# zipnn/zipnn

Hardware: NVIDIA H100
Metric: compress+decompress GB/s on bf16 tensors (higher is better)
Workload: dtype u8

## Files before the change

__graft_entry__.py:

```python
import os
import sys

ROOT = os.path.dirname(os.path.abspath(__file__))
if ROOT not in sys.path:
    sys.path.insert(0, ROOT)


def build() -> None:
    from zipnn_b200 import _native
    _native.build()
    from oracle import oracle as O
    O.build(ref=True)
    import subprocess
    emu = os.path.join(ROOT, "tests", "host_emu")
    subprocess.check_call(["g++", "-O2", "-shared", "-fPIC", "-o", os.path.join(emu, "libemu_serial.so"),
                           os.path.join(emu, "emu_serial.cpp")])
    import zipnn_b200
    _native.lib()


def smoke() -> None:
    import numpy as np
    import torch
    from oracle import oracle as O
    from zipnn_b200 import ZipNN, _native

    assert torch.cuda.is_available(), "smoke() needs a GPU"
    before = _native.launch_count()
    rng = np.random.default_rng(1234)
    for dt, n in ((torch.bfloat16, 300001), (torch.float32, 70001), (torch.float16, 4099), (torch.float8_e4m3fn, 200000)):
        x = torch.from_numpy(rng.standard_normal(n, dtype=np.float32) * np.float32(0.02 if dt != torch.float8_e4m3fn else 0.5)).to(dt)
        z = ZipNN(input_format="torch")
        stream = z.compress(x.cuda())
        plan = ZipNN(input_format="torch").plan(x)
        raw = x.contiguous().view(torch.uint8).numpy()
        want = O.zipnn_compress(plan["header"], raw, plan["num_buf"], plan["bit_reorder"], plan["byte_reorder"],
                                plan["chunk"], plan["threshold"], threads=2)
        got = stream.cpu().numpy()
        assert got.size == want.size and np.array_equal(got, want), f"stream mismatch for {dt}"
        back = ZipNN(input_format="torch").decompress(stream)
        assert back.is_cuda and back.dtype == dt
        assert np.array_equal(back.cpu().contiguous().view(torch.uint8).numpy(), raw), f"round trip mismatch for {dt}"
    torch.cuda.synchronize()
    launched = _native.launch_count() - before
    assert launched > 0
    print(f"smoke ok: 4 dtypes byte-exact vs oracle, {launched} kernel launches from libzipnn_b200.so")


if __name__ == "__main__":
# ... 4 lines not shown
```

zipnn_b200/csrc/api_compress.inc:

```

namespace {
constexpr size_t kHdrMax = 4096;
struct EncWs {
  size_t hdr_off, types_off, sizes_off, itemoff_off, saves_off, part_off, part_bytes, hist_off, total;
};
inline EncWs enc_ws_layout(size_t n, int G, size_t chunk) {
  EncWs L;
  const uint64_t nitems = (uint64_t)G * num_chunks(n, chunk);
  L.hdr_off = kCtrlBytes;
  L.types_off = L.hdr_off + kHdrMax;
  L.sizes_off = round_up(L.types_off + nitems, 256);
  L.itemoff_off = round_up(L.sizes_off + 4 * nitems, 256);
  L.saves_off = round_up(L.itemoff_off + 8 * nitems, 256);
  L.part_off = round_up(L.saves_off + sizeof(EncSave) * nitems, 256);
  L.part_bytes = 8 * (size_t)G * ((num_chunks(n, chunk) + kScanItems - 1) / kScanItems);
  L.hist_off = round_up(L.part_off + L.part_bytes, 256);
  L.total = L.hist_off + 2048 * nitems + 256;
  return L;
}

template <int G>
int launch_encode(const uint8_t* in, size_t n, uint32_t chunk, uint64_t K, int bits_mode, double thr, uint8_t* ws,
                  const EncWs& L, uint32_t hdr_len, uint8_t* out, cudaStream_t st) {
  Ctrl* ctrl = (Ctrl*)ws;
  uint8_t* types = ws + L.types_off;
  uint32_t* sizes = (uint32_t*)(ws + L.sizes_off);
  uint64_t* item_off = (uint64_t*)(ws + L.itemoff_off);
  EncSave* saves = (EncSave*)(ws + L.saves_off);
  const int sms = sm_count_cached();
  uint16_t* hist = (uint16_t*)(ws + L.hist_off);
  {
    const size_t smem = sizeof(HistSmem<G>);
    int per_sm = 1;
    if (smem > 48 * 1024) ZB_CUDA(cudaFuncSetAttribute(k_encode_hist<G>, cudaFuncAttributeMaxDynamicSharedMemorySize, (int)smem));
    ZB_CUDA(cudaOccupancyMaxActiveBlocksPerMultiprocessor(&per_sm, k_encode_hist<G>, kEncThreads, smem));
    if (per_sm < 1) per_sm = 1;
    const int blocks = (int)std::min<uint64_t>(K, (uint64_t)sms * per_sm);
    ScopedTimer tm(kKEncodeStats, st);
    k_encode_hist<G><<<blocks, kEncThreads, smem, st>>>(in, n, chunk, K, bits_mode, hist);
    ZB_LAUNCHED();
  }
  {
    const size_t smem = sizeof(TableWarp) * kTableWarps;
    const uint64_t nitems = (uint64_t)G * K;
    const int blocks = (int)std::min<uint64_t>((nitems + kTableWarps - 1) / kTableWarps, (uint64_t)sms * 16);
    ScopedTimer tm(kKEncodeTable, st);
    ZB_CUDA(cudaMemsetAsync(ws + L.part_off, 0, L.part_bytes, st));
    k_encode_table<G><<<blocks, kTableWarps * 32, smem, st>>>(hist, n, chunk, K, thr, types, sizes, saves,
                                                              (unsigned long long*)(ws + L.part_off));
    ZB_LAUNCHED();
  }
  {
    ScopedTimer tm(kKEncodeScan, st);
    const unsigned nblk = (unsigned)((K + kScanItems - 1) / kScanItems);
    k_encode_scan<<<(unsigned)G * nblk, kScanThreads, 0, st>>>(sizes, types, G, K, ws + L.hdr_off, hdr_len, out, item_off, ctrl,
                                                            (const unsigned long long*)(ws + L.part_off));
    ZB_LAUNCHED();
  }
  if (chunk % (64u * G) != 0) {
    int per_sm = 1;
    ZB_CUDA(cudaOccupancyMaxActiveBlocksPerMultiprocessor(&per_sm, k_encode_write<G>, kEncThreads, 0));
    if (per_sm < 1) per_sm = 1;
    const int blocks = (int)std::min<uint64_t>((uint64_t)G * K, (uint64_t)sms * per_sm);
    ScopedTimer tm(kKEncodeWriteRagged, st);
    k_encode_write<G><<<blocks, kEncThreads, 0, st>>>(in, n, chunk, K, bits_mode, types, sizes, saves, item_off, out, 0);
    ZB_LAUNCHED();
    return ZIPNN_B200_OK;
  }
  {
    int per_sm = 1;
    ZB_CUDA(cudaOccupancyMaxActiveBlocksPerMultiprocessor(&per_sm, k_encode_write_warp<G>, kWbWarps * 32, 0));
    if (per_sm < 1) per_sm = 1;
    const int blocks = (int)std::min<uint64_t>(K, (uint64_t)sms * per_sm);
    ScopedTimer tm(kKEncodeWrite, st);
    k_encode_write_warp<G><<<blocks, kWbWarps * 32, 0, st>>>(in, n, chunk, K, bits_mode, types, sizes, saves, item_off, out);
    ZB_LAUNCHED();
  }
  if ((n % chunk) % (64u * G) != 0) {
// ... 134 lines not shown
    L.part_at[i] = at;
    at += items[i].n ? enc_ws_layout(items[i].n, items[i].num_buf, items[i].chunk).part_bytes : 0;
  }
  L.zero_bytes = at - L.ctrl_off;
  at = round_up(at, 256);
  for (int i = 0; i < n; i++) {
    L.slice_at[i] = at;
    if (items[i].n) {
      const EncWs W = enc_ws_layout(items[i].n, items[i].num_buf, items[i].chunk);
      at += round_up(is_single(i) ? W.total : W.total - W.types_off, 256);
    }
  }
  L.total = at;
  return ZIPNN_B200_OK;
}

template <int G>
int launch_encode_batch(const EncTensor* d_t, uint32_t m, const uint64_t* d_start, const uint64_t* h_start, cudaStream_t st) {
  auto batch = [&](int q) { EncBatch b; b.t = d_t; b.start = d_start + (size_t)q * (m + 1); b.n = m; return b; };
  auto total = [&](int q) { return h_start[(size_t)q * (m + 1) + m]; };
  const int sms = sm_count_cached();
  {
    const size_t smem = sizeof(HistSmem<G>);
    int per_sm = 1;
    if (smem > 48 * 1024) ZB_CUDA(cudaFuncSetAttribute(k_encode_hist_batch<G>, cudaFuncAttributeMaxDynamicSharedMemorySize, (int)smem));
    ZB_CUDA(cudaOccupancyMaxActiveBlocksPerMultiprocessor(&per_sm, k_encode_hist_batch<G>, kEncThreads, smem));
    if (per_sm < 1) per_sm = 1;
    const int blocks = (int)std::max<uint64_t>(1, std::min<uint64_t>(total(0), (uint64_t)sms * per_sm));
    ScopedTimer tm(kKEncodeStats, st);
    k_encode_hist_batch<G><<<blocks, kEncThreads, smem, st>>>(batch(0));
    ZB_LAUNCHED();
  }
  {
    const size_t smem = sizeof(TableWarp) * kTableWarps;
    const int blocks = (int)std::max<uint64_t>(1, std::min<uint64_t>((total(1) + kTableWarps - 1) / kTableWarps, (uint64_t)sms * 16));
    ScopedTimer tm(kKEncodeTable, st);
    k_encode_table_batch<G><<<blocks, kTableWarps * 32, smem, st>>>(batch(1));
    ZB_LAUNCHED();
  }
  {
    ScopedTimer tm(kKEncodeScan, st);
    k_encode_scan_batch<<<(unsigned)total(2), kScanThreads, 0, st>>>(batch(2));
    ZB_LAUNCHED();
  }
  {
    int per_sm = 1;
    ZB_CUDA(cudaOccupancyMaxActiveBlocksPerMultiprocessor(&per_sm, k_encode_write_warp<G, EncBatch>, kWbWarps * 32, 0));
    if (per_sm < 1) per_sm = 1;
    const int blocks = (int)std::max<uint64_t>(1, std::min<uint64_t>(total(3), (uint64_t)sms * per_sm));
    ScopedTimer tm(kKEncodeWrite, st);
    k_encode_write_warp<G, EncBatch><<<blocks, kWbWarps * 32, 0, st>>>(nullptr, 0, 0, 0, 0, nullptr, nullptr, nullptr, nullptr, nullptr, batch(3));
    ZB_LAUNCHED();
  }
  if (total(4)) {
    int per_sm = 1;
    ZB_CUDA(cudaOccupancyMaxActiveBlocksPerMultiprocessor(&per_sm, k_encode_write<G, EncBatch>, kEncThreads, 0));
    if (per_sm < 1) per_sm = 1;
    const int blocks = (int)std::min<uint64_t>(total(4), (uint64_t)sms * per_sm);
    ScopedTimer tm(kKEncodeWriteRagged, st);
    k_encode_write<G, EncBatch><<<blocks, kEncThreads, 0, st>>>(nullptr, 0, 0, 0, 0, nullptr, nullptr, nullptr, nullptr, nullptr, 0, batch(4));
    ZB_LAUNCHED();
  }
  return ZIPNN_B200_OK;
}
}

extern "C" int zipnn_b200_compress_batch_workspace_size(const zipnn_b200_compress_item* items, int n, size_t* out) {
  if (!out) return ZIPNN_B200_E_ARG;
// ... 86 lines not shown
```

zipnn_b200/csrc/encode.cuh:

```cuda
#pragma once
#include "common.cuh"
#include "stage1.cuh"

#include <type_traits>

namespace zb {

struct EncSave {
  uint8_t nb[256];
  uint8_t hdr[128];
  uint32_t hsize;
  uint32_t sbytes[4];
  uint32_t lg;
  uint32_t pad[2];
};
static_assert(sizeof(EncSave) == 416, "EncSave layout");

constexpr int kEncThreads = 256;

struct EncTensor {
  const uint8_t* in;
  uint8_t* out;
  const uint8_t* hdr;
  uint64_t n, K;
  uint32_t chunk, hdr_len;
  int G, bits_mode;
  double thr;
  Ctrl* ctrl;
  unsigned long long* partials;
  uint8_t* types;
  uint32_t* sizes;
  uint64_t* item_off;
  EncSave* saves;
  uint16_t* hist;
};
// ... 100 lines not shown
      }
      if ((q & 1) == 0) continue;
      __syncthreads();
      for (int g = 0; g < G; g++) {
        uint32_t sum = 0;
#pragma unroll
        for (int r = 0; r < R; r++) {
          const int rr = (r + tid) % R;
          sum += S.rep[g][tid][rr];
          S.rep[g][tid][rr] = 0;
        }
        uint16_t* h = hist + (((uint64_t)g * K + c) * 4 + (q - 1)) * 256 + tid;
        h[0] = (uint16_t)(sum & 0xFFFFu);
        h[256] = (uint16_t)(sum >> 16);
      }
      __syncthreads();
    }
  }
}

template <int G>
__global__ void __launch_bounds__(kEncThreads) k_encode_hist(const uint8_t* __restrict__ in, uint64_t n, uint32_t chunk,
                                                             uint64_t K, int bits_mode, uint16_t* __restrict__ hist) {
  encode_hist<G>(in, n, chunk, K, bits_mode, hist, NoBatch{});
}

template <int G>
__global__ void __launch_bounds__(kEncThreads, G == 1 ? 2 : 3) k_encode_hist_batch(EncBatch B) {
  encode_hist<G>(nullptr, 0, 0, 0, 0, nullptr, B);
}

constexpr uint64_t kScanItems = 2048;

struct __align__(16) TableWarp {
  uint32_t total[256];
  uint8_t nb[256];
  uint8_t nzsym[256];
  TreeScratch tree;
};
constexpr int kTableWarps = 4;

__device__ void warp_block_decision(TableWarp& S, const uint16_t* __restrict__ hist, uint32_t plen, uint32_t cap, double thr,
                                    uint8_t* type_out, uint32_t* size_out, EncSave* save) {
  const int lane = threadIdx.x & 31;
  uint32_t* total = S.total;
  uint32_t largest = 0;
  int max_sym = -1;
  for (int s = lane; s < 256; s += 32) {
    const uint32_t t = (uint32_t)__ldg(hist + s) + __ldg(hist + 256 + s) + __ldg(hist + 512 + s) + __ldg(hist + 768 + s);
    total[s] = t;
    largest = max(largest, t);
    if (t) max_sym = s;
  }
#pragma unroll
  for (int o = 16; o; o >>= 1) {
    largest = max(largest, __shfl_xor_sync(0xffffffffu, largest, o));
    max_sym = max(max_sym, __shfl_xor_sync(0xffffffffu, max_sym, o));
  }
  __syncwarp();
  uint32_t stored = 0;
  bool huf = false;
  if (plen == 0 || plen > (uint32_t)kHufBlockMax) {
  } else if (largest == plen) {
    stored = huf_block_decision(true, nullptr, 0, plen, cap, thr);
    if (stored && lane == 0) {
      save->hdr[0] = (uint8_t)max_sym;
      save->hsize = 0;
    }
  } else if (largest <= (plen >> 7) + 4) {
  } else {
    huf = true;
  }
  if (huf) {
    TreeScratch& T = S.tree;
    uint8_t* nz = S.nzsym;
    int k = 0;
    for (int base = 0; base < 256; base += 32) {
      const int s = base + lane;
      const bool p = total[s] != 0;
      const uint32_t m = __ballot_sync(0xffffffffu, p);
      if (p) nz[k + __popc(m & ((1u << lane) - 1u))] = (uint8_t)s;
      k += __popc(m);
    }
    __syncwarp();
    for (int i = lane; i < k; i += 32) {
      const uint32_t c = total[nz[i]];
      int rank = 0;
      for (int j = 0; j < k; j++) {
        const uint32_t cj = total[nz[j]];
        rank += (cj > c) || (cj == c && j < i);
      }
      T.cnt[rank] = c;
      T.sym[rank] = nz[i];
    }
    __syncwarp();
    int lg = 0, hsize = -1;
    if (lane == 0) {
      const int want = fse_pick_log(kHufLogDefault, plen, (uint32_t)max_sym, 1);
      lg = huf_lengths_from_sorted(T, k - 1, want, S.nb);
      hsize = huf_write_table(T, S.nb, max_sym, lg);
    }
    lg = __shfl_sync(0xffffffffu, lg, 0);
    hsize = __shfl_sync(0xffffffffu, hsize, 0);
    __syncwarp();
    if (hsize > 0 && (uint32_t)hsize + 12 < plen) {
      uint32_t bits[4] = {0, 0, 0, 0};
      for (int s = lane; s <= max_sym; s += 32) {
        const uint32_t l = S.nb[s];
#pragma unroll
        for (int q = 0; q < 4; q++) bits[q] += (uint32_t)__ldg(hist + 256 * q + s) * l;
      }
#pragma unroll
      for (int q = 0; q < 4; q++)
#pragma unroll
        for (int o = 16; o; o >>= 1) bits[q] += __shfl_xor_sync(0xffffffffu, bits[q], o);
      stored = huf_block_decision(false, bits, hsize, plen, cap, thr);
      if (stored) {
        for (int s = lane; s < 256; s += 32) save->nb[s] = S.nb[s];
        for (int i = lane; i < hsize; i += 32) save->hdr[i] = T.hdr[i];
        if (lane == 0) {
          save->hsize = (uint32_t)hsize;
          save->lg = (uint32_t)lg;
#pragma unroll
          for (int q = 0; q < 4; q++) save->sbytes[q] = (bits[q] >> 3) + 1;
        }
      }
    }
  }
  if (lane == 0) {
    *type_out = stored ? 1 : 0;
    *size_out = stored ? stored : plen;
  }
}

template <int G>
__device__ __forceinline__ void encode_table_item(TableWarp& S, const uint16_t* __restrict__ hist, uint64_t n, uint32_t chunk, uint64_t K,
                                                  double thr, uint8_t* types, uint32_t* sizes, EncSave* saves,
                                                  unsigned long long* partials, const int lane, uint64_t item) {
  {
    const int g = (int)(item / K);
    const uint64_t c = item - (uint64_t)g * K;
    const uint32_t chunk_len = (c == K - 1) ? (uint32_t)(n - c * (uint64_t)chunk) : chunk;
    warp_block_decision(S, hist + item * 1024, plane_len(chunk_len, G, g), chunk, thr, types + item, sizes + item, saves + item);
    __syncwarp();
    if (lane == 0) atomicAdd(partials + (uint64_t)g * ((K + kScanItems - 1) / kScanItems) + c / kScanItems, (unsigned long long)sizes[item]);
  }
}

template <int G>
__global__ void __launch_bounds__(kTableWarps * 32) k_encode_table(const uint16_t* __restrict__ hist, uint64_t n, uint32_t chunk,
                                                                   uint64_t K, double thr, uint8_t* types, uint32_t* sizes,
                                                                   EncSave* saves, unsigned long long* partials) {
  extern __shared__ __align__(1024) unsigned char smem_raw[];
  TableWarp& S = reinterpret_cast<TableWarp*>(smem_raw)[threadIdx.x >> 5];
  const int lane = threadIdx.x & 31;
  const uint64_t nitems = (uint64_t)G * K;
  for (uint64_t item = (uint64_t)blockIdx.x * kTableWarps + (threadIdx.x >> 5); item < nitems;
       item += (uint64_t)gridDim.x * kTableWarps)
    encode_table_item<G>(S, hist, n, chunk, K, thr, types, sizes, saves, partials, lane, item);
}

constexpr int kScanThreads = 256;

__device__ __forceinline__ void encode_scan_block(const uint32_t* __restrict__ sizes, const uint8_t* __restrict__ types, int G, uint64_t K,
                                                  const uint8_t* __restrict__ hdr_dev, uint32_t hdr_len, uint8_t* out, uint64_t* item_off,
                                                  Ctrl* ctrl, const unsigned long long* __restrict__ partials, uint32_t bid) {
  __shared__ uint64_t warp_tot[kScanThreads / 32];
  __shared__ uint64_t red[kScanThreads / 32][3];
  const int tid = threadIdx.x, lane = tid & 31, warp = tid >> 5;
  const uint64_t nitems = (uint64_t)G * K;
  const uint64_t nblk = (K + kScanItems - 1) / kScanItems;
  const int g = (int)(bid / nblk);
  const uint64_t blk = bid - (uint64_t)g * nblk;
  uint64_t s_groups = 0, s_blocks = 0, s_all = 0;
  for (uint64_t i = tid; i < (uint64_t)G * nblk; i += kScanThreads) {
    const uint64_t v = partials[i];
    const uint64_t gi = i / nblk;
    s_all += v;
    if (gi < (uint64_t)g) s_groups += v;
    if (gi == (uint64_t)g && i - gi * nblk < blk) s_blocks += v;
  }
#pragma unroll
  for (int o = 16; o; o >>= 1) {
    s_groups += __shfl_xor_sync(0xffffffffu, s_groups, o);
    s_blocks += __shfl_xor_sync(0xffffffffu, s_blocks, o);
    s_all += __shfl_xor_sync(0xffffffffu, s_all, o);
  }
  if (lane == 0) { red[warp][0] = s_groups; red[warp][1] = s_blocks; red[warp][2] = s_all; }
  __syncthreads();
  s_groups = s_blocks = s_all = 0;
  for (int w = 0; w < kScanThreads / 32; w++) { s_groups += red[w][0]; s_blocks += red[w][1]; s_all += red[w][2]; }
// ... 588 lines not shown
            asm volatile("red.shared.or.b32 [%0+4], %1;" ::"r"(sa), "r"(w1) : "memory");
            asm volatile("{ .reg .pred p; setp.ne.u32 p, %1, 0; @p red.shared.or.b32 [%0+8], %1; }" ::"r"(sa), "r"(w2) : "memory");
            off += l[r];
          }
          __syncwarp();
          st[g].B += tile_bits;
          wb_flush(bitbuf, st[g], lane);
        }
      }
        };
    do_tile(std::false_type{}, ntiles - 1);
    for (uint32_t ti = ntiles - 1; ti-- > 0;) do_tile(std::true_type{}, ti);
#pragma unroll
    for (int g = 0; g < G; g++) {
      if (S.item[g].type == 1 && S.item[g].size > 1) {
        uint32_t* bitbuf = S.bitbuf[warp][g];
        if (lane == 0) bitbuf[(st[g].B - 32 * st[g].flushed) >> 5] |= 1u << (st[g].B & 31);
        __syncwarp();
        const uint32_t first_byte = max(4 * st[g].flushed, st[g].a);
        const uint32_t end_byte = st[g].a + S.item[g].sbytes[s];
        for (uint32_t bb = first_byte + lane; bb < end_byte; bb += 32) {
          const uint32_t rel = bb - 4 * st[g].flushed;
          st[g].gaddr[bb - st[g].a] = (uint8_t)(bitbuf[rel >> 2] >> (8 * (rel & 3)));
        }
        __syncwarp();
      }
    }
  }
}

template <int G>
__global__ void __launch_bounds__(kTableWarps * 32) k_encode_table_batch(EncBatch B) {
  extern __shared__ __align__(1024) unsigned char smem_raw[];
  TableWarp& S = reinterpret_cast<TableWarp*>(smem_raw)[threadIdx.x >> 5];
  const int lane = threadIdx.x & 31;
  const uint64_t total = B.start[B.n];
  for (uint64_t w = (uint64_t)blockIdx.x * kTableWarps + (threadIdx.x >> 5); w < total; w += (uint64_t)gridDim.x * kTableWarps) {
    const uint32_t i = batch_find(B.start, B.n, w);
    const EncTensor& T = B.t[i];
    encode_table_item<G>(S, T.hist, T.n, T.chunk, T.K, T.thr, T.types, T.sizes, T.saves, T.partials, lane, w - B.start[i]);
  }
}

__global__ void __launch_bounds__(kScanThreads) k_encode_scan_batch(EncBatch B) {
  const uint32_t i = batch_find(B.start, B.n, blockIdx.x);
  const EncTensor& T = B.t[i];
  if (T.K == 0) {
    for (uint32_t j = threadIdx.x; j < T.hdr_len; j += kScanThreads)
      T.out[j] = (j >= 24 && j < 32) ? (uint8_t)((uint64_t)T.hdr_len >> (8 * (j - 24))) : T.hdr[j];
    if (threadIdx.x == 0) T.ctrl->total_len = T.hdr_len;
    return;
  }
  encode_scan_block(T.sizes, T.types, T.G, T.K, T.hdr, T.hdr_len, T.out, T.item_off, T.ctrl, T.partials,
                    (uint32_t)(blockIdx.x - B.start[i]));
}

}
```

zipnn_b200/csrc/huf_serial.cuh:

```cuda
#pragma once
#include <stdint.h>
#include <stddef.h>

#if defined(__CUDACC__)
#define ZB_HD __host__ __device__
#else
#define ZB_HD
#endif

namespace zb {

constexpr int kHufLogMax = 12;
constexpr int kHufLogDefault = 11;
constexpr int kHufBlockMax = 128 * 1024;

ZB_HD inline int hb32(uint32_t v) {
#if defined(__CUDA_ARCH__)
  return 31 - __clz((int)v);
#else
  return 31 - __builtin_clz(v);
#endif
}

struct BitSink {
// ... 85 lines not shown
    int best = 0;
    uint32_t best_c = 0;
    for (int s = 0; s <= max_sym; s++)
      if (count[s] > best_c) {
        best = s;
        best_c = count[s];
      }
    norm[best] = (int16_t)(norm[best] + (int16_t)todo);
    return 0;
  }
  if (total == 0) {
    for (int s = 0; todo > 0; s = (s + 1) % (max_sym + 1))
      if (norm[s] > 0) {
        todo--;
        norm[s]++;
      }
    return 0;
  }
  const int vlog = 62 - lg;
  const uint64_t mid = (1ull << (vlog - 1)) - 1;
  const uint64_t rstep = (((1ull << vlog) * todo) + mid) / total;
  uint64_t acc = mid;
  for (int s = 0; s <= max_sym; s++)
    if (norm[s] == kPending) {
      uint64_t end = acc + (uint64_t)count[s] * rstep;
      uint32_t w = (uint32_t)(end >> vlog) - (uint32_t)(acc >> vlog);
      if (w < 1) return -1;
      norm[s] = (int16_t)w;
      acc = end;
    }
  return 0;
}

ZB_HD inline int fse_normalize(int16_t* norm, int lg, const uint32_t* count, uint32_t total, int max_sym) {
  const uint32_t kRestToBeat[8] = {0, 473195, 504333, 520860, 550000, 700000, 750000, 830000};
  if (lg < 5 || lg > 12) return -1;
  if (lg < fse_min_log(total, (uint32_t)max_sym)) return -1;
  const int scale = 62 - lg;
  const uint64_t step = (1ull << 62) / total;
  const uint64_t vstep = 1ull << (scale - 20);
  int left = 1 << lg;
  int largest = 0;
  int16_t largest_p = 0;
  const uint32_t low_thr = total >> lg;
  for (int s = 0; s <= max_sym; s++) {
    uint32_t c = count[s];
    if (c == total) return 0;
    if (c == 0) {
      norm[s] = 0;
      continue;
    }
    if (c <= low_thr) {
      norm[s] = -1;
      left--;
    } else {
      int16_t p = (int16_t)(((uint64_t)c * step) >> scale);
      if (p < 8) {
        uint64_t beat = vstep * kRestToBeat[p];
        if (((uint64_t)c * step) - ((uint64_t)p << scale) > beat) p++;
      }
      if (p > largest_p) {
        largest_p = p;
        largest = s;
      }
      norm[s] = p;
      left -= p;
    }
  }
  if (-left >= (norm[largest] >> 1)) return fse_normalize_slow(norm, lg, count, total, max_sym);
  norm[largest] = (int16_t)(norm[largest] + left);
  return 0;
}

ZB_HD inline int fse_write_ncount(uint8_t* out, const int16_t* norm, int max_sym, int lg) {
  uint8_t* p = out;
  int remaining = (1 << lg) + 1;
  int threshold = 1 << lg;
  int nbits = lg + 1;
  uint32_t acc = (uint32_t)(lg - 5);
  int cnt = 4;
  int sym = 0;
  const int alphabet = max_sym + 1;
  bool prev0 = false;
  while (sym < alphabet && remaining > 1) {
    if (prev0) {
      int start = sym;
      while (sym < alphabet && norm[sym] == 0) sym++;
      if (sym == alphabet) break;
      while (sym >= start + 24) {
        start += 24;
        acc += 0xFFFFu << cnt;
// ... 72 lines not shown
  }
  uint32_t total = 0;
  for (int s = 0; s <= max_sym; s++) {
    int n = E.norm[s];
    if (n == 0) {
      E.delta_bits[s] = ((uint32_t)(lg + 1) << 16) - size;
      E.delta_find[s] = 0;
    } else if (n == -1 || n == 1) {
      E.delta_bits[s] = ((uint32_t)lg << 16) - size;
      E.delta_find[s] = (int32_t)total - 1;
      total++;
    } else {
      uint32_t max_out = (uint32_t)lg - (uint32_t)hb32((uint32_t)(n - 1));
      uint32_t min_plus = (uint32_t)n << max_out;
      E.delta_bits[s] = (max_out << 16) - min_plus;
      E.delta_find[s] = (int32_t)total - n;
      total += (uint32_t)n;
    }
  }
}

ZB_HD inline uint32_t fse_seed_state(const FseEnc& E, int sym) {
  uint32_t nb = (E.delta_bits[sym] + (1u << 15)) >> 16;
  uint32_t v = (nb << 16) - E.delta_bits[sym];
  return E.next_state[(int32_t)(v >> nb) + E.delta_find[sym]];
}

ZB_HD inline uint32_t fse_step(BitSink& w, const FseEnc& E, uint32_t state, int sym) {
  uint32_t nb = (state + E.delta_bits[sym]) >> 16;
  w.put(state & ((1u << nb) - 1u), (int)nb);
  return E.next_state[(int32_t)(state >> nb) + E.delta_find[sym]];
}

ZB_HD inline int huf_pack_weights(uint8_t* dst, const uint8_t* w, int n, FseEnc& E) {
  if (n <= 1) return 0;
  for (int i = 0; i < 16; i++) E.count[i] = 0;
  int max_w = 0;
  for (int i = 0; i < n; i++) {
    E.count[w[i]]++;
    if (w[i] > max_w) max_w = w[i];
  }
  uint32_t top = 0;
  for (int s = 0; s <= max_w; s++)
    if (E.count[s] > top) top = E.count[s];
  if (top == (uint32_t)n) return 1;
  if (top == 1) return 0;
  const int lg = fse_pick_log(6, (uint32_t)n, (uint32_t)max_w, 2);
  if (fse_normalize(E.norm, lg, E.count, (uint32_t)n, max_w) != 0) return -1;
  int h = fse_write_ncount(dst, E.norm, max_w, lg);
  if (h < 0) return -1;
  fse_build_enc(E, max_w, lg);
  if (n <= 2) return 0;
  BitSink bw;
  bw.init(dst + h);
  int ip = n;
  uint32_t s1, s2;
  if (n & 1) {
    s1 = fse_seed_state(E, w[--ip]);
    s2 = fse_seed_state(E, w[--ip]);
    s1 = fse_step(bw, E, s1, w[--ip]);
  } else {
    s2 = fse_seed_state(E, w[--ip]);
    s1 = fse_seed_state(E, w[--ip]);
  }
  while (ip > 0) {
    s2 = fse_step(bw, E, s2, w[--ip]);
    s1 = fse_step(bw, E, s1, w[--ip]);
  }
  bw.put(s2 & ((1u << lg) - 1u), lg);
  bw.put(s1 & ((1u << lg) - 1u), lg);
  return h + (int)bw.finish();
}

struct TreeScratch {
  uint32_t cnt[512];
  uint16_t parent[512];
  uint8_t depth[512];
  uint8_t sym[256];
  uint8_t weight[256];
  uint8_t hdr[256];
  FseEnc fse;
};

ZB_HD inline int huf_limit_depth(TreeScratch& T, int last, int max_nb) {
  const int deepest = T.depth[last];
  if (deepest <= max_nb) return deepest;
  const uint32_t kNone = 0xF0F0F0F0u;
  int debt = 0;
  const int base = 1 << (deepest - max_nb);
  int n = last;
  while (T.depth[n] > max_nb) {
    debt += base - (1 << (deepest - T.depth[n]));
    T.depth[n] = (uint8_t)max_nb;
    n--;
  }
  while (T.depth[n] == max_nb) n--;
  debt >>= (deepest - max_nb);

  uint32_t rank_last[16];
  for (int i = 0; i < 16; i++) rank_last[i] = kNone;
  {
    int cur = max_nb;
    for (int pos = n; pos >= 0; pos--) {
      if (T.depth[pos] >= cur) continue;
      cur = T.depth[pos];
      rank_last[max_nb - cur] = (uint32_t)pos;
    }
  }
  while (debt > 0) {
    int dec = hb32((uint32_t)debt) + 1;
    for (; dec > 1; dec--) {
      uint32_t hi = rank_last[dec], lo = rank_last[dec - 1];
      if (hi == kNone) continue;
      if (lo == kNone) break;
      if (T.cnt[hi] <= 2 * T.cnt[lo]) break;
    }
    while (dec <= kHufLogMax && rank_last[dec] == kNone) dec++;
    debt -= 1 << (dec - 1);
    if (rank_last[dec - 1] == kNone) rank_last[dec - 1] = rank_last[dec];
    T.depth[rank_last[dec]]++;
    if (rank_last[dec] == 0) {
      rank_last[dec] = kNone;
    } else {
      rank_last[dec]--;
      if (T.depth[rank_last[dec]] != max_nb - dec) rank_last[dec] = kNone;
    }
  }
  while (debt < 0) {
    if (rank_last[1] == kNone) {
      while (T.depth[n] == max_nb) n--;
      T.depth[n + 1]--;
      rank_last[1] = (uint32_t)(n + 1);
      debt++;
      continue;
    }
    T.depth[rank_last[1] + 1]--;
    rank_last[1]++;
    debt++;
  }
  return max_nb;
}

ZB_HD inline int huf_lengths_from_sorted(TreeScratch& T, int last, int max_nb, uint8_t* nb_out) {
  const int kFirst = 256;
  const uint32_t kWall = 0x80000000u;
  int low_leaf = last, low_int = kFirst, next = kFirst;
  const int root = kFirst + last - 1;
  T.cnt[next] = T.cnt[low_leaf] + T.cnt[low_leaf - 1];
  T.parent[low_leaf] = T.parent[low_leaf - 1] = (uint16_t)next;
  next++;
  low_leaf -= 2;
  for (int n = next; n <= root; n++) T.cnt[n] = 1u << 30;
  while (next <= root) {
    uint32_t cl = low_leaf >= 0 ? T.cnt[low_leaf] : kWall;
    int a = (cl < T.cnt[low_int]) ? low_leaf-- : low_int++;
    cl = low_leaf >= 0 ? T.cnt[low_leaf] : kWall;
    int b = (cl < T.cnt[low_int]) ? low_leaf-- : low_int++;
    T.cnt[next] = T.cnt[a] + T.cnt[b];
    T.parent[a] = T.parent[b] = (uint16_t)next;
    next++;
  }
  T.depth[root] = 0;
  for (int n = root - 1; n >= kFirst; n--) T.depth[n] = (uint8_t)(T.depth[T.parent[n]] + 1);
  for (int n = 0; n <= last; n++) T.depth[n] = (uint8_t)(T.depth[T.parent[n]] + 1);
  const int lg = huf_limit_depth(T, last, max_nb);
  for (int s = 0; s < 256; s++) nb_out[s] = 0;
  for (int n = 0; n <= last; n++) nb_out[T.sym[n]] = T.depth[n];
  return lg;
}

ZB_HD inline int huf_sort_serial(TreeScratch& T, const uint32_t* count, int max_sym) {
  int k = 0;
  for (int s = 0; s <= max_sym; s++) {
    uint32_t c = count[s];
    if (c == 0) continue;
    int pos = k++;
    while (pos > 0 && c > T.cnt[pos - 1]) {
      T.cnt[pos] = T.cnt[pos - 1];
      T.sym[pos] = T.sym[pos - 1];
      pos--;
    }
    T.cnt[pos] = c;
    T.sym[pos] = (uint8_t)s;
  }
  return k - 1;
}

ZB_HD inline void huf_assign_values(const uint8_t* nb, int max_sym, int lg, uint16_t* val) {
  uint16_t per_len[kHufLogMax + 2], start[kHufLogMax + 2];
  for (int i = 0; i < kHufLogMax + 2; i++) per_len[i] = start[i] = 0;
  for (int s = 0; s <= max_sym; s++) per_len[nb[s]]++;
  per_len[0] = 0;
  uint16_t v = 0;
  for (int l = lg; l > 0; l--) {
    start[l] = v;
    v = (uint16_t)(v + per_len[l]);
    v >>= 1;
  }
// ... 259 lines not shown
```

Baseline: 526.4.

## Parallelize Huffman table construction across half-warp lane groups

Replaces the lane-0 serial Huffman tree, weight FSE normalization, encoding-table build and bitstream packing with cooperative 16-lane versions, and runs two table items per warp. The smaller shared-memory TableWarp and an occupancy query set the grid size for the table kernels. This targets the serial per-chunk table stage in compression, at the cost of more warp-synchronous code and some remaining serial sections such as tree merging and the FSE state walk. A host emulator is also built for testing.

```diff
diff --git a/__graft_entry__.py b/__graft_entry__.py
--- a/__graft_entry__.py
+++ b/__graft_entry__.py
@@ -13,8 +13,9 @@
     O.build(ref=True)
     import subprocess
     emu = os.path.join(ROOT, "tests", "host_emu")
-    subprocess.check_call(["g++", "-O2", "-shared", "-fPIC", "-o", os.path.join(emu, "libemu_serial.so"),
-                           os.path.join(emu, "emu_serial.cpp")])
+    for name in ("emu_serial", "emu_warp"):
+        subprocess.check_call(["g++", "-O2", "-shared", "-fPIC", "-o", os.path.join(emu, f"lib{name}.so"),
+                               os.path.join(emu, f"{name}.cpp")])
     import zipnn_b200
     _native.lib()
 
diff --git a/zipnn_b200/csrc/api_compress.inc b/zipnn_b200/csrc/api_compress.inc
--- a/zipnn_b200/csrc/api_compress.inc
+++ b/zipnn_b200/csrc/api_compress.inc
@@ -41,9 +41,12 @@
     ZB_LAUNCHED();
   }
   {
-    const size_t smem = sizeof(TableWarp) * kTableWarps;
+    const size_t smem = sizeof(TableWarp) * kTableGroups;
     const uint64_t nitems = (uint64_t)G * K;
-    const int blocks = (int)std::min<uint64_t>((nitems + kTableWarps - 1) / kTableWarps, (uint64_t)sms * 16);
+    int per_sm = 1;
+    ZB_CUDA(cudaOccupancyMaxActiveBlocksPerMultiprocessor(&per_sm, k_encode_table<G>, kTableWarps * 32, smem));
+    if (per_sm < 1) per_sm = 1;
+    const int blocks = (int)std::min<uint64_t>((nitems + kTableGroups - 1) / kTableGroups, (uint64_t)sms * per_sm);
     ScopedTimer tm(kKEncodeTable, st);
     ZB_CUDA(cudaMemsetAsync(ws + L.part_off, 0, L.part_bytes, st));
     k_encode_table<G><<<blocks, kTableWarps * 32, smem, st>>>(hist, n, chunk, K, thr, types, sizes, saves,
@@ -244,8 +247,11 @@
     ZB_LAUNCHED();
   }
   {
-    const size_t smem = sizeof(TableWarp) * kTableWarps;
-    const int blocks = (int)std::max<uint64_t>(1, std::min<uint64_t>((total(1) + kTableWarps - 1) / kTableWarps, (uint64_t)sms * 16));
+    const size_t smem = sizeof(TableWarp) * kTableGroups;
+    int per_sm = 1;
+    ZB_CUDA(cudaOccupancyMaxActiveBlocksPerMultiprocessor(&per_sm, k_encode_table_batch<G>, kTableWarps * 32, smem));
+    if (per_sm < 1) per_sm = 1;
+    const int blocks = (int)std::max<uint64_t>(1, std::min<uint64_t>((total(1) + kTableGroups - 1) / kTableGroups, (uint64_t)sms * per_sm));
     ScopedTimer tm(kKEncodeTable, st);
     k_encode_table_batch<G><<<blocks, kTableWarps * 32, smem, st>>>(batch(1));
     ZB_LAUNCHED();
diff --git a/zipnn_b200/csrc/encode.cuh b/zipnn_b200/csrc/encode.cuh
--- a/zipnn_b200/csrc/encode.cuh
+++ b/zipnn_b200/csrc/encode.cuh
@@ -1,6 +1,7 @@
 #pragma once
 #include "common.cuh"
 #include "stage1.cuh"
+#include "huf_warp.cuh"
 
 #include <type_traits>
 
@@ -167,32 +168,26 @@
 
 constexpr uint64_t kScanItems = 2048;
 
-struct __align__(16) TableWarp {
-  uint32_t total[256];
-  uint8_t nb[256];
-  uint8_t nzsym[256];
-  TreeScratch tree;
-};
 constexpr int kTableWarps = 4;
+constexpr int kTableGroups = kTableWarps * 32 / kTableLanes;
+using TableLanes = CudaWarp<kTableLanes>;
 
 __device__ void warp_block_decision(TableWarp& S, const uint16_t* __restrict__ hist, uint32_t plen, uint32_t cap, double thr,
                                     uint8_t* type_out, uint32_t* size_out, EncSave* save) {
-  const int lane = threadIdx.x & 31;
-  uint32_t* total = S.total;
+  const TableLanes w(threadIdx.x & 31);
+  const int lane = w.lane;
+  uint32_t* total = S.tree.cnt + 256;
   uint32_t largest = 0;
   int max_sym = -1;
-  for (int s = lane; s < 256; s += 32) {
+  for (int s = lane; s < 256; s += kTableLanes) {
     const uint32_t t = (uint32_t)__ldg(hist + s) + __ldg(hist + 256 + s) + __ldg(hist + 512 + s) + __ldg(hist + 768 + s);
     total[s] = t;
     largest = max(largest, t);
     if (t) max_sym = s;
   }
-#pragma unroll
-  for (int o = 16; o; o >>= 1) {
-    largest = max(largest, __shfl_xor_sync(0xffffffffu, largest, o));
-    max_sym = max(max_sym, __shfl_xor_sync(0xffffffffu, max_sym, o));
-  }
-  __syncwarp();
+  largest = warp_max(w, largest);
+  max_sym = (int)warp_max(w, (uint32_t)(max_sym + 1)) - 1;
+  w.sync();
   uint32_t stored = 0;
   bool huf = false;
   if (plen == 0 || plen > (uint32_t)kHufBlockMax) {
@@ -208,51 +203,21 @@
   }
   if (huf) {
     TreeScratch& T = S.tree;
-    uint8_t* nz = S.nzsym;
-    int k = 0;
-    for (int base = 0; base < 256; base += 32) {
-      const int s = base + lane;
-      const bool p = total[s] != 0;
-      const uint32_t m = __ballot_sync(0xffffffffu, p);
-      if (p) nz[k + __popc(m & ((1u << lane) - 1u))] = (uint8_t)s;
-      k += __popc(m);
-    }
-    __syncwarp();
-    for (int i = lane; i < k; i += 32) {
-      const uint32_t c = total[nz[i]];
-      int rank = 0;
-      for (int j = 0; j < k; j++) {
-        const uint32_t cj = total[nz[j]];
-        rank += (cj > c) || (cj == c && j < i);
-      }
-      T.cnt[rank] = c;
-      T.sym[rank] = nz[i];
-    }
-    __syncwarp();
-    int lg = 0, hsize = -1;
-    if (lane == 0) {
-      const int want = fse_pick_log(kHufLogDefault, plen, (uint32_t)max_sym, 1);
-      lg = huf_lengths_from_sorted(T, k - 1, want, S.nb);
-      hsize = huf_write_table(T, S.nb, max_sym, lg);
-    }
-    lg = __shfl_sync(0xffffffffu, lg, 0);
-    hsize = __shfl_sync(0xffffffffu, hsize, 0);
-    __syncwarp();
+    int lg = 0;
+    const int hsize = warp_huf_table(w, S, plen, max_sym, &lg);
     if (hsize > 0 && (uint32_t)hsize + 12 < plen) {
       uint32_t bits[4] = {0, 0, 0, 0};
-      for (int s = lane; s <= max_sym; s += 32) {
+      for (int s = lane; s <= max_sym; s += kTableLanes) {
         const uint32_t l = S.nb[s];
 #pragma unroll
         for (int q = 0; q < 4; q++) bits[q] += (uint32_t)__ldg(hist + 256 * q + s) * l;
       }
 #pragma unroll
-      for (int q = 0; q < 4; q++)
-#pragma unroll
-        for (int o = 16; o; o >>= 1) bits[q] += __shfl_xor_sync(0xffffffffu, bits[q], o);
+      for (int q = 0; q < 4; q++) bits[q] = warp_sum(w, bits[q]);
       stored = huf_block_decision(false, bits, hsize, plen, cap, thr);
       if (stored) {
-        for (int s = lane; s < 256; s += 32) save->nb[s] = S.nb[s];
-        for (int i = lane; i < hsize; i += 32) save->hdr[i] = T.hdr[i];
+        for (int s = lane; s < 256; s += kTableLanes) save->nb[s] = S.nb[s];
+        for (int i = lane; i < hsize; i += kTableLanes) save->hdr[i] = T.hdr[i];
         if (lane == 0) {
           save->hsize = (uint32_t)hsize;
           save->lg = (uint32_t)lg;
@@ -277,7 +242,7 @@
     const uint64_t c = item - (uint64_t)g * K;
     const uint32_t chunk_len = (c == K - 1) ? (uint32_t)(n - c * (uint64_t)chunk) : chunk;
     warp_block_decision(S, hist + item * 1024, plane_len(chunk_len, G, g), chunk, thr, types + item, sizes + item, saves + item);
-    __syncwarp();
+    TableLanes(threadIdx.x & 31).sync();
     if (lane == 0) atomicAdd(partials + (uint64_t)g * ((K + kScanItems - 1) / kScanItems) + c / kScanItems, (unsigned long long)sizes[item]);
   }
 }
@@ -287,11 +252,11 @@
                                                                    uint64_t K, double thr, uint8_t* types, uint32_t* sizes,
                                                                    EncSave* saves, unsigned long long* partials) {
   extern __shared__ __align__(1024) unsigned char smem_raw[];
-  TableWarp& S = reinterpret_cast<TableWarp*>(smem_raw)[threadIdx.x >> 5];
-  const int lane = threadIdx.x & 31;
+  TableWarp& S = reinterpret_cast<TableWarp*>(smem_raw)[threadIdx.x / kTableLanes];
+  const int lane = threadIdx.x % kTableLanes;
   const uint64_t nitems = (uint64_t)G * K;
-  for (uint64_t item = (uint64_t)blockIdx.x * kTableWarps + (threadIdx.x >> 5); item < nitems;
-       item += (uint64_t)gridDim.x * kTableWarps)
+  for (uint64_t item = (uint64_t)blockIdx.x * kTableGroups + threadIdx.x / kTableLanes; item < nitems;
+       item += (uint64_t)gridDim.x * kTableGroups)
     encode_table_item<G>(S, hist, n, chunk, K, thr, types, sizes, saves, partials, lane, item);
 }
 
@@ -946,10 +911,10 @@
 template <int G>
 __global__ void __launch_bounds__(kTableWarps * 32) k_encode_table_batch(EncBatch B) {
   extern __shared__ __align__(1024) unsigned char smem_raw[];
-  TableWarp& S = reinterpret_cast<TableWarp*>(smem_raw)[threadIdx.x >> 5];
-  const int lane = threadIdx.x & 31;
+  TableWarp& S = reinterpret_cast<TableWarp*>(smem_raw)[threadIdx.x / kTableLanes];
+  const int lane = threadIdx.x % kTableLanes;
   const uint64_t total = B.start[B.n];
-  for (uint64_t w = (uint64_t)blockIdx.x * kTableWarps + (threadIdx.x >> 5); w < total; w += (uint64_t)gridDim.x * kTableWarps) {
+  for (uint64_t w = (uint64_t)blockIdx.x * kTableGroups + threadIdx.x / kTableLanes; w < total; w += (uint64_t)gridDim.x * kTableGroups) {
     const uint32_t i = batch_find(B.start, B.n, w);
     const EncTensor& T = B.t[i];
     encode_table_item<G>(S, T.hist, T.n, T.chunk, T.K, T.thr, T.types, T.sizes, T.saves, T.partials, lane, w - B.start[i]);
diff --git a/zipnn_b200/csrc/huf_serial.cuh b/zipnn_b200/csrc/huf_serial.cuh
--- a/zipnn_b200/csrc/huf_serial.cuh
+++ b/zipnn_b200/csrc/huf_serial.cuh
@@ -141,8 +141,20 @@
   return 0;
 }
 
+ZB_HD inline uint32_t fse_rest_to_beat(int p) {
+  switch (p) {
+    case 0: return 0;
+    case 1: return 473195;
+    case 2: return 504333;
+    case 3: return 520860;
+    case 4: return 550000;
+    case 5: return 700000;
+    case 6: return 750000;
+    default: return 830000;
+  }
+}
+
 ZB_HD inline int fse_normalize(int16_t* norm, int lg, const uint32_t* count, uint32_t total, int max_sym) {
-  const uint32_t kRestToBeat[8] = {0, 473195, 504333, 520860, 550000, 700000, 750000, 830000};
   if (lg < 5 || lg > 12) return -1;
   if (lg < fse_min_log(total, (uint32_t)max_sym)) return -1;
   const int scale = 62 - lg;
@@ -165,7 +177,7 @@
     } else {
       int16_t p = (int16_t)(((uint64_t)c * step) >> scale);
       if (p < 8) {
-        uint64_t beat = vstep * kRestToBeat[p];
+        uint64_t beat = vstep * fse_rest_to_beat(p);
         if (((uint64_t)c * step) - ((uint64_t)p << scale) > beat) p++;
       }
       if (p > largest_p) {
@@ -304,6 +316,28 @@
   return E.next_state[(int32_t)(state >> nb) + E.delta_find[sym]];
 }
 
+ZB_HD inline int fse_encode_weights(uint8_t* dst, const uint8_t* w, int n, const FseEnc& E, int lg) {
+  BitSink bw;
+  bw.init(dst);
+  int ip = n;
+  uint32_t s1, s2;
+  if (n & 1) {
+    s1 = fse_seed_state(E, w[--ip]);
+    s2 = fse_seed_state(E, w[--ip]);
+    s1 = fse_step(bw, E, s1, w[--ip]);
+  } else {
+    s2 = fse_seed_state(E, w[--ip]);
+    s1 = fse_seed_state(E, w[--ip]);
+  }
+  while (ip > 0) {
+    s2 = fse_step(bw, E, s2, w[--ip]);
+    s1 = fse_step(bw, E, s1, w[--ip]);
+  }
+  bw.put(s2 & ((1u << lg) - 1u), lg);
+  bw.put(s1 & ((1u << lg) - 1u), lg);
+  return (int)bw.finish();
+}
+
 ZB_HD inline int huf_pack_weights(uint8_t* dst, const uint8_t* w, int n, FseEnc& E) {
   if (n <= 1) return 0;
   for (int i = 0; i < 16; i++) E.count[i] = 0;
@@ -323,25 +357,7 @@
   if (h < 0) return -1;
   fse_build_enc(E, max_w, lg);
   if (n <= 2) return 0;
-  BitSink bw;
-  bw.init(dst + h);
-  int ip = n;
-  uint32_t s1, s2;
-  if (n & 1) {
-    s1 = fse_seed_state(E, w[--ip]);
-    s2 = fse_seed_state(E, w[--ip]);
-    s1 = fse_step(bw, E, s1, w[--ip]);
-  } else {
-    s2 = fse_seed_state(E, w[--ip]);
-    s1 = fse_seed_state(E, w[--ip]);
-  }
-  while (ip > 0) {
-    s2 = fse_step(bw, E, s2, w[--ip]);
-    s1 = fse_step(bw, E, s1, w[--ip]);
-  }
-  bw.put(s2 & ((1u << lg) - 1u), lg);
-  bw.put(s1 & ((1u << lg) - 1u), lg);
-  return h + (int)bw.finish();
+  return h + fse_encode_weights(dst + h, w, n, E, lg);
 }
 
 struct TreeScratch {
@@ -354,7 +370,7 @@
   FseEnc fse;
 };
 
-ZB_HD inline int huf_limit_depth(TreeScratch& T, int last, int max_nb) {
+ZB_HD inline int huf_limit_depth(TreeScratch& T, int last, int max_nb, uint32_t* rank_last) {
   const int deepest = T.depth[last];
   if (deepest <= max_nb) return deepest;
   const uint32_t kNone = 0xF0F0F0F0u;
@@ -369,7 +385,6 @@
   while (T.depth[n] == max_nb) n--;
   debt >>= (deepest - max_nb);
 
-  uint32_t rank_last[16];
   for (int i = 0; i < 16; i++) rank_last[i] = kNone;
   {
     int cur = max_nb;
@@ -435,7 +450,8 @@
   T.depth[root] = 0;
   for (int n = root - 1; n >= kFirst; n--) T.depth[n] = (uint8_t)(T.depth[T.parent[n]] + 1);
   for (int n = 0; n <= last; n++) T.depth[n] = (uint8_t)(T.depth[T.parent[n]] + 1);
-  const int lg = huf_limit_depth(T, last, max_nb);
+  uint32_t rank_last[16];
+  const int lg = huf_limit_depth(T, last, max_nb, rank_last);
   for (int s = 0; s < 256; s++) nb_out[s] = 0;
   for (int n = 0; n <= last; n++) nb_out[T.sym[n]] = T.depth[n];
   return lg;
diff --git a/zipnn_b200/csrc/huf_warp.cuh b/zipnn_b200/csrc/huf_warp.cuh
--- /dev/null
+++ b/zipnn_b200/csrc/huf_warp.cuh
@@ -0,0 +1,404 @@
+#pragma once
+#include "huf_serial.cuh"
+
+#if defined(__CUDACC__)
+#define ZB_WARP_FN __device__
+#else
+#define ZB_WARP_FN
+#endif
+
+namespace zb {
+
+struct alignas(16) TableWarp {
+  uint8_t nb[256];
+  uint8_t nzsym[256];
+  TreeScratch tree;
+  uint32_t rank_last[16];
+};
+
+constexpr int kTableLanes = 16;
+
+#if defined(__CUDACC__)
+template <int LANES>
+struct CudaWarp {
+  static constexpr int kLanes = LANES;
+  int lane;
+  int base;
+  uint32_t mask;
+  __device__ __forceinline__ explicit CudaWarp(int warp_lane)
+      : lane(warp_lane % LANES), base(warp_lane - warp_lane % LANES),
+        mask((LANES == 32 ? 0xffffffffu : ((1u << (LANES % 32)) - 1u)) << (warp_lane - warp_lane % LANES)) {}
+  __device__ __forceinline__ uint32_t shfl(uint32_t v, int src) const { return __shfl_sync(mask, v, src, LANES); }
+  __device__ __forceinline__ uint32_t shfl_xor(uint32_t v, int m) const { return __shfl_xor_sync(mask, v, m, LANES); }
+  __device__ __forceinline__ uint32_t ballot(bool p) const { return (__ballot_sync(mask, p) & mask) >> base; }
+  __device__ __forceinline__ uint32_t match_any(uint32_t v) const { return (__match_any_sync(mask, v) & mask) >> base; }
+  __device__ __forceinline__ void sync() const { __syncwarp(mask); }
+  __device__ __forceinline__ void or_shared(uint32_t* p, uint32_t v) const { atomicOr(p, v); }
+};
+#endif
+
+ZB_HD inline int popc32(uint32_t v) {
+#if defined(__CUDA_ARCH__)
+  return __popc(v);
+#else
+  return __builtin_popcount(v);
+#endif
+}
+
+template <class W>
+ZB_WARP_FN inline uint32_t warp_sum(const W& w, uint32_t v) {
+  for (int o = W::kLanes / 2; o; o >>= 1) v += w.shfl_xor(v, o);
+  return v;
+}
+template <class W>
+ZB_WARP_FN inline uint32_t warp_max(const W& w, uint32_t v) {
+  for (int o = W::kLanes / 2; o; o >>= 1) {
+    const uint32_t u = w.shfl_xor(v, o);
+    v = u > v ? u : v;
+  }
+  return v;
+}
+
+template <class W>
+ZB_WARP_FN inline int warp_sort_symbols(const W& w, TableWarp& S) {
+  TreeScratch& T = S.tree;
+  uint32_t* const cz = T.cnt + 256;
+  const int lane = w.lane;
+  int k = 0;
+  for (int base = 0; base < 256; base += W::kLanes) {
+    const uint32_t c = cz[base + lane];
+    const uint32_t m = w.ballot(c != 0);
+    if (c) {
+      const int i = k + popc32(m & ((1u << lane) - 1u));
+      cz[i] = c;
+      S.nzsym[i] = (uint8_t)(base + lane);
+    }
+    k += popc32(m);
+  }
+  w.sync();
+  for (int i = lane; i < k; i += W::kLanes) {
+    const uint32_t c = cz[i];
+    int rank = 0;
+    for (int j = 0; j < k; j++) {
+      const uint32_t cj = cz[j];
+      rank += (cj > c) || (cj == c && j < i);
+    }
+    T.cnt[rank] = c;
+    T.sym[rank] = S.nzsym[i];
+  }
+  w.sync();
+  return k;
+}
+
+template <class W>
+ZB_WARP_FN inline int warp_lengths_from_sorted(const W& w, TableWarp& S, int last, int max_nb) {
+  TreeScratch& T = S.tree;
+  const int lane = w.lane;
+  const int kFirst = 256;
+  const int root = kFirst + last - 1;
+  if (lane == 0) {
+    const uint32_t kWall = 0x80000000u, kEmpty = 1u << 30;
+    int low_leaf = last - 2, low_int = kFirst, next = kFirst + 1;
+    uint32_t sum = T.cnt[last] + T.cnt[last - 1];
+    T.cnt[kFirst] = sum;
+    T.parent[last] = T.parent[last - 1] = (uint16_t)kFirst;
+    uint32_t cl = low_leaf >= 0 ? T.cnt[low_leaf] : kWall;
+    uint32_t ci = sum;
+    while (next <= root) {
+      int a, b;
+      uint32_t ca, cb;
+      if (cl < ci) {
+        a = low_leaf--; ca = cl;
+        cl = low_leaf >= 0 ? T.cnt[low_leaf] : kWall;
+      } else {
+        a = low_int++; ca = ci;
+        ci = low_int < next ? T.cnt[low_int] : kEmpty;
+      }
+      if (cl < ci) {
+        b = low_leaf--; cb = cl;
+        cl = low_leaf >= 0 ? T.cnt[low_leaf] : kWall;
+      } else {
+        b = low_int++; cb = ci;
+        ci = low_int < next ? T.cnt[low_int] : kEmpty;
+      }
+      sum = ca + cb;
+      T.cnt[next] = sum;
+      T.parent[a] = T.parent[b] = (uint16_t)next;
+      if (low_int == next) ci = sum;
+      next++;
+    }
+    T.depth[root] = 0;
+    for (int n = root - 1; n >= kFirst; n--) T.depth[n] = (uint8_t)(T.depth[T.parent[n]] + 1);
+  }
+  for (int i = lane; i < 64; i += W::kLanes) reinterpret_cast<uint32_t*>(S.nb)[i] = 0;
+  w.sync();
+  for (int n = lane; n <= last; n += W::kLanes) T.depth[n] = (uint8_t)(T.depth[T.parent[n]] + 1);
+  w.sync();
+  int lg = (int)w.shfl(T.depth[last], 0);
+  if (lg > max_nb) {
+    if (lane == 0) huf_limit_depth(T, last, max_nb, S.rank_last);
+    lg = max_nb;
+    w.sync();
+  }
+  for (int n = lane; n <= last; n += W::kLanes) S.nb[T.sym[n]] = T.depth[n];
+  w.sync();
+  return lg;
+}
+
+template <class W>
+ZB_WARP_FN inline int warp_fse_normalize(const W& w, int16_t* norm, int lg, const uint32_t* count, uint32_t total, int max_sym) {
+  if (lg < 5 || lg > 12) return -1;
+  if (lg < fse_min_log(total, (uint32_t)max_sym)) return -1;
+  const int lane = w.lane;
+  const int scale = 62 - lg;
+  const uint64_t step = (1ull << 62) / total;
+  const uint64_t vstep = 1ull << (scale - 20);
+  const uint32_t low_thr = total >> lg;
+  const uint32_t c = lane <= max_sym ? count[lane] : 0;
+  int nv = 0;
+  uint32_t used = 0, key = 0;
+  if (c != 0 && c <= low_thr) {
+    nv = -1;
+    used = 1;
+  } else if (c != 0) {
+    int p = (int)(((uint64_t)c * step) >> scale);
+    if (p < 8) {
+      const uint64_t beat = vstep * fse_rest_to_beat(p);
+      if (((uint64_t)c * step) - ((uint64_t)p << scale) > beat) p++;
+    }
+    nv = p;
+    used = (uint32_t)p;
+    key = ((uint32_t)p << 5) | (uint32_t)(31 - lane);
+  }
+  if (lane <= max_sym) norm[lane] = (int16_t)nv;
+  const int left = (1 << lg) - (int)warp_sum(w, used);
+  key = warp_max(w, key);
+  const int largest = key ? 31 - (int)(key & 31u) : 0;
+  w.sync();
+  const int nl = norm[largest];
+  int rc = 0;
+  if (-left >= (nl >> 1)) {
+    w.sync();
+    if (lane == 0) rc = fse_normalize_slow(norm, lg, count, total, max_sym);
+    rc = (int)w.shfl((uint32_t)rc, 0);
+  } else {
+    w.sync();
+    if (lane == largest) norm[largest] = (int16_t)(nl + left);
+  }
+  w.sync();
+  return rc;
+}
+
+template <class W>
+ZB_WARP_FN inline void warp_fse_build_enc(const W& w, FseEnc& E, int max_sym, int lg) {
+  const int lane = w.lane;
+  const uint32_t size = 1u << lg, mask = size - 1;
+  const uint32_t step = (size >> 1) + (size >> 3) + 3;
+  const uint32_t lt = (1u << lane) - 1u;
+  const int n = lane <= max_sym ? E.norm[lane] : 0;
+  const uint32_t cells = n == -1 ? 1u : (uint32_t)n;
+  const uint32_t spread_n = n > 0 ? (uint32_t)n : 0u;
+  uint32_t cum = cells, walk = spread_n;
+  for (int o = 1; o < W::kLanes; o <<= 1) {
+    const uint32_t a = w.shfl(cum, lane - o), b = w.shfl(walk, lane - o);
+    if (lane >= o) { cum += a; walk += b; }
+  }
+  const uint32_t before = cum - cells;
+  if (lane < 16) E.count[lane] = 0;
+  if (lane <= max_sym) {
+    E.cumul[lane] = before;
+    if (n == 0) {
+      E.delta_bits[lane] = ((uint32_t)(lg + 1) << 16) - size;
+      E.delta_find[lane] = 0;
+    } else if (n == -1 || n == 1) {
+      E.delta_bits[lane] = ((uint32_t)lg << 16) - size;
+      E.delta_find[lane] = (int32_t)before - 1;
+    } else {
+      const uint32_t max_out = (uint32_t)lg - (uint32_t)hb32((uint32_t)(n - 1));
+      E.delta_bits[lane] = (max_out << 16) - ((uint32_t)n << max_out);
+      E.delta_find[lane] = (int32_t)before - n;
+    }
+  }
+  const uint32_t low = w.ballot(n == -1);
+  const uint32_t high = size - 1 - (uint32_t)popc32(low);
+  if (n == -1) E.spread[size - 1 - (uint32_t)popc32(low & lt)] = (uint8_t)lane;
+  uint32_t kept = 0;
+  for (uint32_t base = 0; base < size; base += W::kLanes) {
+    const uint32_t pos = ((base + (uint32_t)lane) * step) & mask;
+    const bool keep = pos <= high;
+    const uint32_t km = w.ballot(keep);
+    const uint32_t i = kept + (uint32_t)popc32(km & lt);
+    kept += (uint32_t)popc32(km);
+    uint32_t sym = 0;
+    for (int s = 0; s < max_sym; s++) sym += (i >= w.shfl(walk, s));
+    if (keep) E.spread[pos] = (uint8_t)sym;
+  }
+  w.sync();
+  for (uint32_t base = 0; base < size; base += W::kLanes) {
+    const uint32_t u = base + (uint32_t)lane;
+    const uint32_t s = E.spread[u];
+    const uint32_t same = w.match_any(s);
+    const uint32_t slot = E.cumul[s] + E.count[s] + (uint32_t)popc32(same & lt);
+    w.sync();
+    E.next_state[slot] = (uint16_t)(size + u);
+    if ((same & lt) == 0) E.count[s] += (uint32_t)popc32(same);
+    w.sync();
+  }
+}
+
+template <class W>
+ZB_WARP_FN inline int warp_encode_weights(const W& w, TableWarp& S, uint8_t* dst, int n, int lg) {
+  TreeScratch& T = S.tree;
+  const FseEnc& E = T.fse;
+  const int lane = w.lane;
+  uint32_t* const db = T.cnt;
+  int32_t* const df = reinterpret_cast<int32_t*>(T.cnt + 256);
+  uint16_t* const rec = T.parent;
+  for (int i = lane; i < n; i += W::kLanes) {
+    const int wt = T.weight[i];
+    db[i] = E.delta_bits[wt];
+    df[i] = E.delta_find[wt];
+  }
+  w.sync();
+  int r = 0;
+  if (lane == 0) {
+    const uint16_t* const ns = E.next_state;
+    auto seed = [&](int i) -> uint32_t {
+      const uint32_t nb = (db[i] + (1u << 15)) >> 16;
+      return ns[(int32_t)(((nb << 16) - db[i]) >> nb) + df[i]];
+    };
+    auto step = [&](uint32_t st, int i) -> uint32_t {
+      const uint32_t nb = (st + db[i]) >> 16;
+      rec[r++] = (uint16_t)((st << 4) | nb);
+      return ns[(int32_t)(st >> nb) + df[i]];
+    };
+    int ip = n;
+    uint32_t s1, s2;
+    if (n & 1) {
+      s1 = seed(--ip);
+      s2 = seed(--ip);
+      s1 = step(s1, --ip);
+    } else {
+      s2 = seed(--ip);
+      s1 = seed(--ip);
+    }
+    while (ip > 0) {
+      s2 = step(s2, --ip);
+      s1 = step(s1, --ip);
+    }
+    const uint32_t m = (1u << lg) - 1u;
+    rec[r++] = (uint16_t)(((s2 & m) << 4) | (uint32_t)lg);
+    rec[r++] = (uint16_t)(((s1 & m) << 4) | (uint32_t)lg);
+    rec[r++] = (uint16_t)((1u << 4) | 1u);
+  }
+  r = (int)w.shfl((uint32_t)r, 0);
+  w.sync();
+  uint32_t* const buf = T.cnt;
+  for (int i = lane; i < 64; i += W::kLanes) buf[i] = 0;
+  w.sync();
+  uint32_t total = 0;
+  for (int first = 0; first < r; first += 8 * W::kLanes) {
+    uint64_t bits = 0;
+    uint32_t nbits = 0;
+    for (int j = 0; j < 8; j++) {
+      const int i = first + 8 * lane + j;
+      if (i < r) {
+        const uint32_t v = rec[i], nb = v & 15u;
+        bits |= (uint64_t)((v >> 4) & ((1u << nb) - 1u)) << nbits;
+        nbits += nb;
+      }
+    }
+    uint32_t end = nbits;
+    for (int o = 1; o < W::kLanes; o <<= 1) {
+      const uint32_t t = w.shfl(end, lane - o);
+      if (lane >= o) end += t;
+    }
+    const uint32_t off = total + end - nbits, sh = off & 31u;
+    total += w.shfl(end, W::kLanes - 1);
+    if (nbits) {
+      w.or_shared(buf + (off >> 5), (uint32_t)(bits << sh));
+      w.or_shared(buf + (off >> 5) + 1, (uint32_t)(bits >> (32u - sh)));
+      if (sh) w.or_shared(buf + (off >> 5) + 2, (uint32_t)(bits >> (64u - sh)));
+    }
+  }
+  w.sync();
+  const int bytes = (int)((total + 7u) >> 3);
+  for (int i = lane; i < bytes; i += W::kLanes) dst[i] = reinterpret_cast<const uint8_t*>(buf)[i];
+  return bytes;
+}
+
+template <class W>
+ZB_WARP_FN inline int warp_write_table(const W& w, TableWarp& S, int max_sym, int lg) {
+  TreeScratch& T = S.tree;
+  FseEnc& E = T.fse;
+  const int lane = w.lane;
+  const int n = max_sym;
+  if (lane < 16) E.count[lane] = 0;
+  w.sync();
+  uint32_t max_w = 0;
+  for (int base = 0; base < n; base += W::kLanes) {
+    const int s = base + lane;
+    uint32_t wt = 0xFFu;
+    if (s < n) {
+      const uint32_t l = S.nb[s];
+      wt = l ? (uint32_t)(lg + 1) - l : 0u;
+      T.weight[s] = (uint8_t)wt;
+      max_w = wt > max_w ? wt : max_w;
+    }
+    const uint32_t same = w.match_any(wt);
+    if (s < n && (same & ((1u << lane) - 1u)) == 0) E.count[wt] += (uint32_t)popc32(same);
+    w.sync();
+  }
+  max_w = warp_max(w, max_w);
+  const uint32_t top = warp_max(w, lane < 16 ? E.count[lane] : 0u);
+  int h;
+  if (n <= 1) {
+    h = 0;
+  } else if (top == (uint32_t)n) {
+    h = 1;
+  } else if (top == 1) {
+    h = 0;
+  } else {
+    const int lg6 = fse_pick_log(6, (uint32_t)n, max_w, 2);
+    h = warp_fse_normalize(w, E.norm, lg6, E.count, (uint32_t)n, (int)max_w);
+    if (h == 0) {
+      if (lane == 0) {
+        h = fse_write_ncount(T.hdr + 1, E.norm, (int)max_w, lg6);
+        if (h >= 0 && n <= 2) h = 0;
+      }
+      h = (int)w.shfl((uint32_t)h, 0);
+      w.sync();
+      if (h > 0) {
+        warp_fse_build_enc(w, E, (int)max_w, lg6);
+        h += warp_encode_weights(w, S, T.hdr + 1 + h, n, lg6);
+      }
+    }
+  }
+  w.sync();
+  if (h < 0) return -1;
+  if (h > 1 && h < n / 2) {
+    if (lane == 0) T.hdr[0] = (uint8_t)h;
+    w.sync();
+    return h + 1;
+  }
+  if (n > 128) return -1;
+  if (lane == 0) {
+    T.hdr[0] = (uint8_t)(128 + (n - 1));
+    T.weight[n] = 0;
+  }
+  w.sync();
+  for (int s = 2 * lane; s < n; s += 2 * W::kLanes) T.hdr[(s / 2) + 1] = (uint8_t)((T.weight[s] << 4) + T.weight[s + 1]);
+  w.sync();
+  return ((n + 1) / 2) + 1;
+}
+
+template <class W>
+ZB_WARP_FN inline int warp_huf_table(const W& w, TableWarp& S, uint32_t plen, int max_sym, int* lg_out) {
+  const int k = warp_sort_symbols(w, S);
+  const int want = fse_pick_log(kHufLogDefault, plen, (uint32_t)max_sym, 1);
+  const int lg = warp_lengths_from_sorted(w, S, k - 1, want);
+  *lg_out = lg;
+  return warp_write_table(w, S, max_sym, lg);
+}
+
+}
```

After: 534.2 (median of 6 runs). No clear change (+1.5%).
